# danihae/bio-image-unet

Hardware: AMD Instinct MI355X
Metric: voxels/sec fwd+bwd (higher is better)
Workload: dtype bf16; 1 GPU; cfg4: UNet3D(in_channels=1, out_channels=1, n_filter=32) input (4, 1, 128, 128, 128) per GPU, train step = forward + reference loss + backward + Adam; parallelism=dp1

## Files before the change

### bio_image_unet_amd/csrc/biu_api.hip

```cpp
#include "biu_common.h"
#include "biu_internal.h"

#include <stdlib.h>
#include <string.h>

static const char* const kOffTokens[] = {
    "conv_fwd", "conv_dgrad", "conv_wgrad", "convt_fwd", "convt_dgrad", "convt_wgrad", "convt_all", "c1", "c1_mfma", "cat",
    "fused_stats", "wgrad_bn", "dgrad_bnred", "pool_pair", "pool_pipe", "pool_bnred", "head_bnred", "ksplit", "m16", "m16x2", "rr16",
    "wroll", "wroll16", "wroll2d", "upconv", "foldt", "foldall", "foldck8", "foldgemm", "croll", "froll", "prepack", "wsplitbn",
    "capturefork", "sidechain", "headrank1",
};
constexpr int kNumOffTokens = sizeof(kOffTokens) / sizeof(kOffTokens[0]);
static_assert(kNumOffTokens <= 64, "BiuEnv::off holds one bit per token");

static int off_index(const char* tok, size_t n) {
    for (int i = 0; i < kNumOffTokens; ++i)
        if (strlen(kOffTokens[i]) == n && strncmp(kOffTokens[i], tok, n) == 0) return i;
    return -1;
}
static void env_unknown(const char* var, const char* val, int n) {
    fprintf(stderr, "[biu] %s: unknown %s '%.*s' ignored\n", var, strcmp(var, "BIU_DISABLE") == 0 ? "token" : "value", n, val);
}
static bool parse_int(const char* s, int* v) {
    char* end = nullptr;
    const long r = strtol(s, &end, 10);
    if (end == s || *end) return false;
    *v = (int)r;
    return true;
}

const BiuEnv& biu_env() {
    static const BiuEnv env = [] {
        BiuEnv v{0, false, false, 0, 2, 0, 128};
        if (const char* p = getenv("BIU_DISABLE")) {
            while (true) {
                const size_t n = strcspn(p, ",");
                const int i = off_index(p, n);
                if (i >= 0) v.off |= 1ull << i;
                else if (n > 0) env_unknown("BIU_DISABLE", p, (int)n);
                if (!p[n]) break;
                p += n + 1;
            }
        }
// ... 539 lines not shown
```

### bio_image_unet_amd/csrc/biu_c1.hip

```cpp
#include "biu_internal.h"
#include <stdlib.h>
#include <string.h>

namespace {

typedef float floatx16 __attribute__((ext_vector_type(16)));
typedef __bf16 bf16x8 __attribute__((ext_vector_type(8)));
typedef __bf16 bf16x4 __attribute__((ext_vector_type(4)));
typedef unsigned u32x2 __attribute__((ext_vector_type(2)));

constexpr int ROWB = 80;

struct C1Args {
    const char* x; int xpitch;
    char* y; int ypitch;
    const char* yraw; int yrawpitch;
    const float* w;
    const float* bias;
    const float* xs; const float* xb; const float* xl;
    int N, D, H, W, co0, cout;
    int nbd, nbh, nbw, nbricks;
    float* partial;
    int ctot;
    const float* bn_scale; const float* bn_shift; const float* bn_slope; const float* bn_cA; const float* bn_cB; const float* bn_cC;
};

__device__ __forceinline__ unsigned pack2(float a, float b) {
    typedef __bf16 bf2 __attribute__((ext_vector_type(2)));
    const bf2 p = {(__bf16)a, (__bf16)b};
    return __builtin_bit_cast(unsigned, p);
}
__device__ __forceinline__ void unpack8(const uint4& v, float* f) {
    const unsigned u[4] = {v.x, v.y, v.z, v.w};
#pragma unroll
    for (int i = 0; i < 4; ++i) { f[2 * i] = __uint_as_float(u[i] << 16); f[2 * i + 1] = __uint_as_float(u[i] & 0xffff0000u); }
}
__device__ __forceinline__ float bf2f(unsigned short u) { return __uint_as_float((unsigned)u << 16); }

template <int KD, int HALF = 0> struct Geo {
    static constexpr int TD = (KD == 3) ? (HALF ? 1 : 2) : 1, TH = (KD == 3) ? 8 : (HALF ? 8 : 16), TW = 32;
    static constexpr int BV = TD * TH * TW;
    static constexpr int HD = TD + KD - 1, HH = TH + 2, HW = TW + 2;
    static constexpr int HV = HD * HH * HW;
    static constexpr int TAPS = KD * 9;
};

template <int KD, int NTHR, int HALF = 0>
struct XpRegs { unsigned short v[(Geo<KD, HALF>::HV + NTHR - 1) / NTHR]; unsigned inside; };

template <int KD, int NTHR, int HALF = 0>
__device__ __forceinline__ void xp_request(const C1Args& a, int n, int d0, int h0, int w0, XpRegs<KD, NTHR, HALF>& xr) {
    using G = Geo<KD, HALF>;
    constexpr int NX = (G::HV + NTHR - 1) / NTHR;
    const int tid = threadIdx.x;
    xr.inside = 0;
#pragma unroll
    for (int k = 0; k < NX; ++k) {
        const int i = tid + NTHR * k;
        const int hw = i % G::HW, t = i / G::HW;
        const int hh = t % G::HH, hd = t / G::HH;
        const int gd = d0 + hd - (KD == 3 ? 1 : 0), gh = h0 + hh - 1, gw = w0 + hw - 1;
        const bool ok = i < G::HV && gd >= 0 && gd < a.D && gh >= 0 && gh < a.H && gw >= 0 && gw < a.W;
        xr.v[k] = ok ? *(const unsigned short*)(a.x + ((size_t)(((size_t)n * a.D + gd) * a.H + gh) * a.W + gw) * a.xpitch * 2) : (unsigned short)0;
        xr.inside |= ok ? (1u << k) : 0u;
    }
}
template <int KD, int NTHR, int HALF = 0>
__device__ __forceinline__ void xp_commit(const C1Args& a, const XpRegs<KD, NTHR, HALF>& xr, unsigned short* lx, char* lxp) {
    using G = Geo<KD, HALF>;
    constexpr int NX = (G::HV + NTHR - 1) / NTHR;
    const int tid = threadIdx.x;
    const bool has_xf = a.xs != nullptr;
    const float xs = has_xf ? a.xs[0] : 1.f, xb = has_xf ? a.xb[0] : 0.f, xl = has_xf ? a.xl[0] : 1.f;
#pragma unroll
    for (int k = 0; k < NX; ++k) {
        const int i = tid + NTHR * k;
        if (i < G::HV) {
            unsigned short v = xr.v[k];
            if (has_xf && ((xr.inside >> k) & 1u)) {
                const float tt = fmaf(xs, bf2f(v), xb);
                const float o = tt > 0.f ? tt : xl * tt;
                v = (unsigned short)(pack2(o, 0.f) & 0xffffu);
            }
            lx[i] = v;
        }
    }
    __syncthreads();
    for (int v = tid; v < G::BV; v += NTHR) {
        const int lw = v % G::TW, t = v / G::TW;
        const int lh = t % G::TH, ld = t / G::TH;
        unsigned short val[32];
#pragma unroll
        for (int tap = 0; tap < 32; ++tap) {
            if (tap < G::TAPS) {
                const int ta = tap / 9, tb = (tap / 3) % 3, tc = tap % 3;
                val[tap] = lx[((ld + ta) * G::HH + (lh + tb)) * G::HW + (lw + tc)];
            } else {
                val[tap] = 0;
            }
        }
        uint4* dst = (uint4*)(lxp + v * ROWB);
#pragma unroll
        for (int q = 0; q < 4; ++q)
            dst[q] = make_uint4(val[8 * q] | ((unsigned)val[8 * q + 1] << 16), val[8 * q + 2] | ((unsigned)val[8 * q + 3] << 16),
                                val[8 * q + 4] | ((unsigned)val[8 * q + 5] << 16), val[8 * q + 6] | ((unsigned)val[8 * q + 7] << 16));
    }
    __syncthreads();
}

template <int KD, int NQ >
__global__ __launch_bounds__(256) void k_c1_fwd_mfma(C1Args a) {
    using G = Geo<KD>;
    __shared__ __attribute__((aligned(16))) char smem[G::BV * ROWB + G::HV * 2 + 16 + 4 * 64 * 4 + 32 * 4];
    char* lxp = smem;
    unsigned short* lx = (unsigned short*)(smem + G::BV * ROWB);
    float* lred = (float*)(smem + G::BV * ROWB + ((G::HV * 2 + 15) & ~15));
    float* lbias = lred + 4 * 64;
    const int tid = threadIdx.x, lane = tid & 63, wave = tid >> 6, r = lane & 31, hf = lane >> 5;
    lred[tid] = 0.f;
    if (tid < 32) lbias[tid] = (a.bias && tid < a.cout) ? a.bias[a.co0 + tid] : 0.f;
    uint4 wf[2];
#pragma unroll
    for (int ks = 0; ks < 2; ++ks) {
        float f[8];
#pragma unroll
        for (int e = 0; e < 8; ++e) {
            const int tap = 16 * ks + 8 * hf + e;
            f[e] = (r < a.cout && tap < G::TAPS) ? a.w[(size_t)(a.co0 + r) * G::TAPS + tap] : 0.f;
        }
        wf[ks] = make_uint4(pack2(f[0], f[1]), pack2(f[2], f[3]), pack2(f[4], f[5]), pack2(f[6], f[7]));
    }
    float s1[NQ][8], s2[NQ][8];
#pragma unroll
    for (int q = 0; q < NQ; ++q)
#pragma unroll
        for (int e = 0; e < 8; ++e) s1[q][e] = s2[q][e] = 0.f;
    __syncthreads();

    auto origin_of = [&](int brick, int& n, int& d0, int& h0, int& w0) {
        int b = brick;
        w0 = (b % a.nbw) * G::TW; b /= a.nbw;
        h0 = (b % a.nbh) * G::TH; b /= a.nbh;
        d0 = (b % a.nbd) * G::TD;
        n = b / a.nbd;
    };
    XpRegs<KD, 256> xr;
    if ((int)blockIdx.x < a.nbricks) { int n, d0, h0, w0; origin_of(blockIdx.x, n, d0, h0, w0); xp_request<KD, 256>(a, n, d0, h0, w0, xr); }
    for (int brick = blockIdx.x; brick < a.nbricks; brick += gridDim.x) {
        int n, d0, h0, w0;
        origin_of(brick, n, d0, h0, w0);
        xp_commit<KD, 256>(a, xr, lx, lxp);
        if (brick + (int)gridDim.x < a.nbricks) { int n2, d2, h2, w2; origin_of(brick + gridDim.x, n2, d2, h2, w2); xp_request<KD, 256>(a, n2, d2, h2, w2, xr); }
        for (int tile = wave; tile < G::BV / 32; tile += 4) {
            const int v = tile * 32 + r;
            floatx16 acc;
#pragma unroll
            for (int e = 0; e < 16; ++e) acc[e] = lbias[8 * (e >> 2) + 4 * hf + (e & 3)];
#pragma unroll
            for (int ks = 0; ks < 2; ++ks) {
                const uint4 bx = *(const uint4*)(lxp + v * ROWB + (16 * ks + 8 * hf) * 2);
                acc = __builtin_amdgcn_mfma_f32_32x32x16_bf16(__builtin_bit_cast(bf16x8, wf[ks]), __builtin_bit_cast(bf16x8, bx), acc, 0, 0, 0);
            }
            const int lw = v % G::TW, t = v / G::TW;
            const int gd = d0 + t / G::TH, gh = h0 + t % G::TH, gw = w0 + lw;
            const bool vok = gd < a.D && gh < a.H && gw < a.W;
            char* orow = a.y + ((size_t)(((size_t)n * a.D + gd) * a.H + gh) * a.W + gw) * a.ypitch * 2;
#pragma unroll
            for (int q = 0; q < NQ; ++q) {
                unsigned a0 = pack2(acc[8 * q + 0], acc[8 * q + 1]), a1 = pack2(acc[8 * q + 2], acc[8 * q + 3]);
                unsigned b0 = pack2(acc[8 * q + 4], acc[8 * q + 5]), b1 = pack2(acc[8 * q + 6], acc[8 * q + 7]);
                const u32x2 r0 = __builtin_amdgcn_permlane32_swap(a0, b0, false, false);
                const u32x2 r1 = __builtin_amdgcn_permlane32_swap(a1, b1, false, false);
                const uint4 piece = make_uint4(r0[0], r1[0], r0[1], r1[1]);
                const int c = 16 * q + 8 * hf;
                if (vok && c < a.cout) {
                    *(uint4*)(orow + (size_t)(a.co0 + c) * 2) = piece;
                    float f[8];
                    unpack8(piece, f);
#pragma unroll
                    for (int e = 0; e < 8; ++e) { s1[q][e] += f[e]; s2[q][e] = fmaf(f[e], f[e], s2[q][e]); }
                }
            }
        }
        __syncthreads();
    }
    if (a.partial) {
#pragma unroll
        for (int q = 0; q < NQ; ++q)
#pragma unroll
            for (int e = 0; e < 8; ++e) {
                float u = s1[q][e], w_ = s2[q][e];
#pragma unroll
                for (int o = 16; o > 0; o >>= 1) { u += __shfl_xor(u, o, 64); w_ += __shfl_xor(w_, o, 64); }
                if (r == 0) { lred[wave * 64 + 2 * (16 * q + 8 * hf + e)] = u; lred[wave * 64 + 2 * (16 * q + 8 * hf + e) + 1] = w_; }
            }
        __syncthreads();
        if (tid < a.cout) {
            float* dst = a.partial + ((size_t)blockIdx.x * a.ctot + a.co0 + tid) * 2;
            dst[0] = (lred[2 * tid] + lred[64 + 2 * tid]) + (lred[128 + 2 * tid] + lred[192 + 2 * tid]);
            dst[1] = (lred[2 * tid + 1] + lred[64 + 2 * tid + 1]) + (lred[128 + 2 * tid + 1] + lred[192 + 2 * tid + 1]);
        }
    }
}

template <int KD>
__global__ __launch_bounds__(256, 3) void k_c1_wgrad_mfma(C1Args a) {
    using G = Geo<KD, 1>;
    constexpr int NTHR = 256, NWV = 4;
    extern __shared__ __attribute__((aligned(16))) char smem[];
    char* lxp = smem;
    char* ldy = smem + G::BV * ROWB;
    unsigned short* lx = (unsigned short*)(ldy + G::BV * ROWB);
    float* lacc = (float*)((char*)lx + ((G::HV * 2 + 15) & ~15));
    const int tid = threadIdx.x, lane = tid & 63, wave = tid >> 6;
    const bool fused = a.yraw != nullptr;
    const int ppv = a.cout / 8;
    const int mypiece = tid % 4;
    float ks[8], kh[8], kl[8], ka[8], kb[8], kc[8];
    if (fused && mypiece < ppv) {
#pragma unroll
        for (int e = 0; e < 8; ++e) {
            const int c = a.co0 + mypiece * 8 + e;
            ks[e] = a.bn_scale[c]; kh[e] = a.bn_shift[c]; kl[e] = a.bn_slope ? a.bn_slope[c] : 1.f;
            ka[e] = a.bn_cA[c]; kb[e] = a.bn_cB[c]; kc[e] = a.bn_cC[c];
        }
    }
    for (int i = tid; i < 32 * 32; i += NTHR) lacc[i] = 0.f;
    floatx16 acc;
#pragma unroll
    for (int e = 0; e < 16; ++e) acc[e] = 0.f;
    const int g = lane >> 4, li = lane & 15, qrow = li >> 2, p = li & 3, cg = g & 1, h = g >> 1;
    const int tr_lane = (8 * h + qrow) * ROWB + (16 * cg + 4 * p) * 2;

    constexpr int NPC = G::BV * 4 / NTHR;
    uint4 pda[NPC], pyr[NPC];
    size_t pvox[NPC];
    unsigned pmask = 0;
    auto origin = [&](int brick, int& n, int& d0, int& h0, int& w0) {
        int b = brick;
        w0 = (b % a.nbw) * G::TW; b /= a.nbw;
        h0 = (b % a.nbh) * G::TH; b /= a.nbh;
        d0 = (b % a.nbd) * G::TD;
        n = b / a.nbd;
    };
    auto request = [&](int brick) {
        int n, d0, h0, w0;
        origin(brick, n, d0, h0, w0);
        pmask = 0;
#pragma unroll
        for (int k = 0; k < NPC; ++k) {
            const int v = (tid + NTHR * k) / 4;
            const int lw = v % G::TW, t = v / G::TW;
            const int gd = d0 + t / G::TH, gh = h0 + t % G::TH, gw = w0 + lw;
            pda[k] = make_uint4(0, 0, 0, 0);
            pyr[k] = make_uint4(0, 0, 0, 0);
            if (mypiece < ppv && gd < a.D && gh < a.H && gw < a.W) {
                const size_t vox = (((size_t)n * a.D + gd) * a.H + gh) * a.W + gw;
                pvox[k] = vox;
                pda[k] = *(const uint4*)(a.y + (vox * a.ypitch + a.co0 + mypiece * 8) * 2);
                if (fused) pyr[k] = *(const uint4*)(a.yraw + (vox * a.yrawpitch + a.co0 + mypiece * 8) * 2);
                pmask |= 1u << k;
            }
        }
    };
    XpRegs<KD, NTHR, 1> xr;
    if ((int)blockIdx.x < a.nbricks) {
        request(blockIdx.x);
        int n0, d00, h00, w00;
        origin(blockIdx.x, n0, d00, h00, w00);
        xp_request<KD, NTHR, 1>(a, n0, d00, h00, w00, xr);
    }
    for (int brick = blockIdx.x; brick < a.nbricks; brick += gridDim.x) {
        int n, d0, h0, w0;
        origin(brick, n, d0, h0, w0);
#pragma unroll
        for (int k = 0; k < NPC; ++k) {
            const int v = (tid + NTHR * k) / 4;
            uint4 out = pda[k];
            if (fused && ((pmask >> k) & 1u)) {
                float gg[8], yy[8];
                unpack8(out, gg);
                unpack8(pyr[k], yy);
#pragma unroll
                for (int e = 0; e < 8; ++e) {
                    const float dz = gg[e] * (fmaf(ks[e], yy[e], kh[e]) > 0.f ? 1.f : kl[e]);
                    gg[e] = fmaf(ka[e], dz, fmaf(kb[e], yy[e], kc[e]));
                }
                out = make_uint4(pack2(gg[0], gg[1]), pack2(gg[2], gg[3]), pack2(gg[4], gg[5]), pack2(gg[6], gg[7]));
                *(uint4*)(a.y + (pvox[k] * a.ypitch + a.co0 + mypiece * 8) * 2) = out;
            }
            *(uint4*)(ldy + v * ROWB + mypiece * 16) = out;
        }
        xp_commit<KD, NTHR, 1>(a, xr, lx, lxp);
        if (brick + (int)gridDim.x < a.nbricks) {
            request(brick + gridDim.x);
            int n2, d2, h2, w2;
            origin(brick + gridDim.x, n2, d2, h2, w2);
            xp_request<KD, NTHR, 1>(a, n2, d2, h2, w2, xr);
        }
        typedef bf16x4 __attribute__((address_space(3))) * lp;
        for (int ksx = wave; ksx < G::BV / 16; ksx += NWV) {
            const char* ap = lxp + ksx * 16 * ROWB + tr_lane;
            const char* bp = ldy + ksx * 16 * ROWB + tr_lane;
            const bf16x4 a0 = __builtin_amdgcn_ds_read_tr16_b64_v4bf16((lp)(ap));
            const bf16x4 a1 = __builtin_amdgcn_ds_read_tr16_b64_v4bf16((lp)(ap + 4 * ROWB));
            const bf16x4 b0 = __builtin_amdgcn_ds_read_tr16_b64_v4bf16((lp)(bp));
            const bf16x4 b1 = __builtin_amdgcn_ds_read_tr16_b64_v4bf16((lp)(bp + 4 * ROWB));
            acc = __builtin_amdgcn_mfma_f32_32x32x16_bf16(__builtin_shufflevector(a0, a1, 0, 1, 2, 3, 4, 5, 6, 7),
                                                          __builtin_shufflevector(b0, b1, 0, 1, 2, 3, 4, 5, 6, 7), acc, 0, 0, 0);
        }
        __syncthreads();
    }
    {
        const int j = lane & 31, hf = lane >> 5;
#pragma unroll
        for (int e = 0; e < 16; ++e) atomicAdd(&lacc[((e & 3) + 8 * (e >> 2) + 4 * hf) * 32 + j], acc[e]);
    }
    __syncthreads();
    for (int i = tid; i < G::TAPS * a.cout; i += NTHR) {
        const int tap = i / a.cout, co = i % a.cout;
        a.partial[(size_t)blockIdx.x * (G::TAPS * a.cout) + i] = lacc[tap * 32 + co];
    }
}

__global__ void k_c1m_finalize(const float* __restrict__ partial, int nblk, int taps, int cout, int co0, float* __restrict__ dw) {
    __shared__ double red[256];
    const int o = blockIdx.x;
    double s = 0;
    for (int b = threadIdx.x; b < nblk; b += 256) s += partial[(size_t)b * (taps * cout) + o];
    red[threadIdx.x] = s;
    __syncthreads();
    for (int st = 128; st > 0; st >>= 1) {
        if (threadIdx.x < st) red[threadIdx.x] += red[threadIdx.x + st];
        __syncthreads();
    }
    if (threadIdx.x == 0) dw[(size_t)(co0 + o % cout) * taps + o / cout] = (float)red[0];
}

int cus() {
    static int n = 0;
    if (!n) {
        hipDeviceProp_t p;
        int dev = 0;
        if (hipGetDevice(&dev) == hipSuccess && hipGetDeviceProperties(&p, dev) == hipSuccess) n = p.multiProcessorCount;
        if (n <= 0) n = 256;
    }
    return n;
}

template <int KD, int HALF = 0> void bricks_of(C1Args& a) {
    using G = Geo<KD, HALF>;
    a.nbd = (a.D + G::TD - 1) / G::TD; a.nbh = (a.H + G::TH - 1) / G::TH; a.nbw = (a.W + G::TW - 1) / G::TW;
    a.nbricks = a.N * a.nbd * a.nbh * a.nbw;
}

}

bool biu_c1m_ok(const biu_act* x, const biu_act* y, int kd, int kh, int kw, int dil, int dtype) {
    if (biu_off("c1_mfma") || dtype != BIU_BF16 || x->c != 1 || dil != 1 || kh != 3 || kw != 3 || (kd != 1 && kd != 3)) return false;
    if (y->c % 16 != 0 || y->c < 16) return false;
    if ((uintptr_t)y->p % 16 || (y->pitch * 2) % 16 || (uintptr_t)x->p % 2) return false;
    return nvox(y) < (1LL << 31);
}

int biu_c1m_fwd_rows(const biu_act* y, int kd) {
    C1Args a{};
    a.N = y->n; a.D = y->d; a.H = y->h; a.W = y->w;
    if (kd == 3) bricks_of<3>(a); else bricks_of<1>(a);
    const int g = 3 * cus();
    return g < a.nbricks ? g : a.nbricks;
}

int biu_c1m_fwd(const biu_act* x, const biu_xform* xf, const float* w, const float* bias, int kd, const biu_act* y, float* bn_partial, hipStream_t st) {
    C1Args a{};
    a.x = (const char*)x->p; a.xpitch = x->pitch; a.y = (char*)y->p; a.ypitch = y->pitch; a.w = w; a.bias = bias;
    if (xf && (xf->scale || xf->shift || xf->slope)) {
        BIU_REQUIRE(xf->scale && xf->shift && xf->slope, BIU_ERR_UNSUPPORTED, "c1 conv: partial biu_xform");
        a.xs = xf->scale; a.xb = xf->shift; a.xl = xf->slope;
    }
    a.N = y->n; a.D = y->d; a.H = y->h; a.W = y->w; a.ctot = y->c; a.partial = bn_partial;
    const int rows = biu_c1m_fwd_rows(y, kd);
    if (kd == 3) bricks_of<3>(a); else bricks_of<1>(a);
    for (int co0 = 0; co0 < y->c;) {
        const int chunk = (y->c - co0) >= 32 ? 32 : 16;
        a.co0 = co0; a.cout = chunk;
        if (kd == 3) { if (chunk == 32) hipLaunchKernelGGL((k_c1_fwd_mfma<3, 2>), dim3(rows), dim3(256), 0, st, a); else hipLaunchKernelGGL((k_c1_fwd_mfma<3, 1>), dim3(rows), dim3(256), 0, st, a); }
        else { if (chunk == 32) hipLaunchKernelGGL((k_c1_fwd_mfma<1, 2>), dim3(rows), dim3(256), 0, st, a); else hipLaunchKernelGGL((k_c1_fwd_mfma<1, 1>), dim3(rows), dim3(256), 0, st, a); }
        co0 += chunk;
    }
    BIU_CHECK_LAUNCH("c1_fwd_mfma");
    return BIU_OK;
}

size_t biu_c1m_wgrad_workspace(int cout, int kd) { return (size_t)3 * cus() * kd * 9 * 32 * sizeof(float); }

int biu_c1m_wgrad(const biu_act* x, const biu_xform* xf, const biu_act* da, const BnBwdFuse* bn, int kd, float* dw, void* ws, size_t ws_bytes,
                  hipStream_t st) {
    BIU_REQUIRE(ws && ws_bytes >= biu_c1m_wgrad_workspace(da->c, kd), BIU_ERR_WORKSPACE, "c1_wgrad_mfma: workspace too small");
    C1Args a{};
    if (xf && (xf->scale || xf->shift || xf->slope)) {
        BIU_REQUIRE(xf->scale && xf->shift && xf->slope, BIU_ERR_UNSUPPORTED, "c1 conv: partial biu_xform");
        a.xs = xf->scale; a.xb = xf->shift; a.xl = xf->slope;
    }
    a.x = (const char*)x->p; a.xpitch = x->pitch; a.y = (char*)da->p; a.ypitch = da->pitch;
    a.N = da->n; a.D = da->d; a.H = da->h; a.W = da->w; a.partial = (float*)ws; a.ctot = da->c;
    if (bn) {
        a.yraw = (const char*)bn->y->p; a.yrawpitch = bn->y->pitch;
        a.bn_scale = bn->scale; a.bn_shift = bn->shift; a.bn_slope = bn->slope; a.bn_cA = bn->cA; a.bn_cB = bn->cB; a.bn_cC = bn->cC;
    }
    const int taps = kd * 9;
    if (kd == 3) bricks_of<3, 1>(a); else bricks_of<1, 1>(a);
    int grid = 3 * cus();
    if (grid > a.nbricks) grid = a.nbricks;
    const size_t hv = kd == 3 ? (size_t)Geo<3, 1>::HV : (size_t)Geo<1, 1>::HV;
    const size_t lds = (size_t)2 * 256 * ROWB + ((hv * 2 + 15) & ~(size_t)15) + 32 * 32 * sizeof(float);
    for (int co0 = 0; co0 < da->c;) {
        const int chunk = (da->c - co0) >= 32 ? 32 : 16;
        a.co0 = co0; a.cout = chunk;
        if (kd == 3) hipLaunchKernelGGL(k_c1_wgrad_mfma<3>, dim3(grid), dim3(256), lds, st, a);
        else hipLaunchKernelGGL(k_c1_wgrad_mfma<1>, dim3(grid), dim3(256), lds, st, a);
        BIU_CHECK_LAUNCH("c1_wgrad_mfma");
        hipLaunchKernelGGL(k_c1m_finalize, dim3(taps * chunk), dim3(256), 0, st, (const float*)ws, grid, taps, chunk, co0, dw);
        BIU_CHECK_LAUNCH("c1_wgrad_mfma_finalize");
        co0 += chunk;
    }
    return BIU_OK;
}
```

### bio_image_unet_amd/csrc/biu_special.hip

```cpp
#include "biu_internal.h"
#include <cstring>
#include <cstdlib>
#include <stdlib.h>

#define TPB 256

struct Vox4 { int n, d, h, w; };
__device__ __forceinline__ Vox4 unvox4(i64 v, int D, int H, int W) {
    Vox4 r;
    if ((unsigned long long)v < (1ull << 32)) {
        unsigned u = (unsigned)v;
        r.w = (int)(u % (unsigned)W); u /= (unsigned)W;
        r.h = (int)(u % (unsigned)H); u /= (unsigned)H;
        r.d = (int)(u % (unsigned)D); u /= (unsigned)D;
        r.n = (int)u;
        return r;
    }
    r.w = (int)(v % W); v /= W;
    r.h = (int)(v % H); v /= H;
    r.d = (int)(v % D); v /= D;
    r.n = (int)v;
    return r;
}

// ... 449 lines not shown
    BIU_CHECK_LAUNCH("bn_bwd_reduce_vec");
    return BIU_OK;
}

__global__ void k_partial_sum0(const float* __restrict__ partial, int nblk, int C, float* __restrict__ out) {
    __shared__ double red[TPB];
    const int c = blockIdx.x;
    double a = 0;
    for (int b = threadIdx.x; b < nblk; b += TPB) a += partial[((i64)b * C + c) * 2];
    red[threadIdx.x] = a;
    __syncthreads();
    for (int s = TPB / 2; s > 0; s >>= 1) {
        if (threadIdx.x < s) red[threadIdx.x] += red[threadIdx.x + s];
        __syncthreads();
    }
    if (threadIdx.x == 0) out[c] = (float)red[0];
}
size_t biu_chan_sum_workspace(int c) { return (size_t)BIU_BN_MAX_PARTIALS * c * 2 * sizeof(float); }
int biu_chan_sum_vec(const biu_act* a, float* out, void* ws, int dtype, hipStream_t st) {
    int nblk = 0;
    BIU_DISPATCH_DTYPE(dtype, {
        constexpr int PE = 16 / sizeof(T);
        VPlan p = vplan(nvox(a), a->c, PE);
        VSum<T> f{dact(a)};
        hipLaunchKernelGGL((k_chan_reduce2_vec<VSum<T>, PE>), dim3(p.nblk), dim3(TPB), p.smem, st, f, nvox(a), a->c, p.ppv, p.vpb, (float*)ws);
        nblk = p.nblk;
    });
    BIU_CHECK_LAUNCH("chan_sum_vec");
    hipLaunchKernelGGL(k_partial_sum0, dim3(a->c), dim3(TPB), 0, st, (const float*)ws, nblk, a->c, out);
    BIU_CHECK_LAUNCH("partial_sum0");
    return BIU_OK;
}

template <typename T, int C, int O, bool RED, bool STORE = true>
__global__ __launch_bounds__(TPB) void k_head_bwd_fused(DAct x, DXf xf, const float* __restrict__ w, int cout,
                                                        const float* __restrict__ dl, DAct dx, int want_dx,
                                                        float* __restrict__ partial ,
                                                        const float* __restrict__ mean, const float* __restrict__ invstd,
                                                        float* __restrict__ bn_partial) {
    constexpr int G = 16 / sizeof(T);
    __shared__ float wsm[O * C];
    __shared__ float xsc[C], xsh[C], xsl[C];
    __shared__ float red[4][O * C + O];
    for (int i = threadIdx.x; i < O * C; i += TPB) wsm[i] = (i / C) < cout ? w[i] : 0.f;
    for (int i = threadIdx.x; i < C; i += TPB) {
        xsc[i] = xf.scale ? xf.scale[i] : 1.f;
        xsh[i] = xf.shift ? xf.shift[i] : 0.f;
        xsl[i] = xf.slope ? xf.slope[i] : 1.f;
    }
    __syncthreads();
    const i64 S = (i64)x.d * x.h * x.w;
    const i64 total = (i64)x.n * S;
    float aw[O][C], ab[O];
    float r1[RED ? C : 1], r2[RED ? C : 1];
#pragma unroll
    for (int o = 0; o < O; ++o) {
        ab[o] = 0.f;
#pragma unroll
        for (int c = 0; c < C; ++c) aw[o][c] = 0.f;
    }
    if (RED) {
#pragma unroll
        for (int c = 0; c < C; ++c) r1[c] = r2[c] = 0.f;
    }
    for (i64 v = (i64)blockIdx.x * TPB + threadIdx.x; v < total; v += (i64)gridDim.x * TPB) {
        const i64 n = v / S, s = v % S;
        float g[O];
#pragma unroll
        for (int o = 0; o < O; ++o) {
            g[o] = (o < cout) ? dl[(n * cout + o) * S + s] : 0.f;
            ab[o] += g[o];
        }
        const T* src = (const T*)x.p + v * x.pitch;
        T* dst = (STORE && want_dx) ? (T*)dx.p + v * dx.pitch : nullptr;
#pragma unroll
        for (int c0 = 0; c0 < C; c0 += G) {
            Pack<T, G> in = *(const Pack<T, G>*)(src + c0);
            Pack<T, G> od;
#pragma unroll
            for (int j = 0; j < G; ++j) {
                const int c = c0 + j;
                float t = fmaf(xsc[c], to_f(in.v[j]), xsh[c]);
                t = t > 0.f ? t : xsl[c] * t;
                float d = 0.f;
#pragma unroll
                for (int o = 0; o < O; ++o) {
                    aw[o][c] = fmaf(g[o], t, aw[o][c]);
                    d = fmaf(g[o], wsm[o * C + c], d);
                }
                od.v[j] = from_f<T>(d);
                if (RED) {
                    const float yv = to_f(in.v[j]);
                    const float dz = to_f(od.v[j]) * (fmaf(xsc[c], yv, xsh[c]) > 0.f ? 1.f : xsl[c]);
                    r1[c] += dz;
                    r2[c] = fmaf(dz, yv, r2[c]);
                }
            }
            if (STORE && want_dx) *(Pack<T, G>*)(dst + c0) = od;
        }
    }
    const int lane = threadIdx.x & 63, wave = threadIdx.x >> 6;
#pragma unroll
    for (int o = 0; o < O; ++o) {
#pragma unroll
        for (int c = 0; c < C; ++c) {
            const float r = wave_sum(aw[o][c]);
            if (lane == 0) red[wave][o * C + c] = r;
        }
        const float rb = wave_sum(ab[o]);
        if (lane == 0) red[wave][O * C + o] = rb;
    }
    __syncthreads();
    for (int i = threadIdx.x; i < O * C + O; i += TPB)
        partial[(i64)blockIdx.x * (O * C + O) + i] = red[0][i] + red[1][i] + red[2][i] + red[3][i];
    if (RED) {
        __shared__ float redb[4][2 * C];
#pragma unroll
        for (int c = 0; c < C; ++c) {
            const float a1 = wave_sum(r1[c]), a2 = wave_sum(r2[c]);
            if (lane == 0) { redb[wave][2 * c] = a1; redb[wave][2 * c + 1] = a2; }
        }
        __syncthreads();
        for (int c = threadIdx.x; c < C; c += TPB) {
            const float s1v = redb[0][2 * c] + redb[1][2 * c] + redb[2][2 * c] + redb[3][2 * c];
            const float s2v = redb[0][2 * c + 1] + redb[1][2 * c + 1] + redb[2][2 * c + 1] + redb[3][2 * c + 1];
            bn_partial[((i64)blockIdx.x * C + c) * 2 + 0] = s1v;
            bn_partial[((i64)blockIdx.x * C + c) * 2 + 1] = invstd[c] * (s2v - mean[c] * s1v);
        }
    }
}

// ... 13 lines not shown
            const int o = i / C, c = i % C;
            if (o < cout && dw) dw[o * C + c] = (float)red[0];
        } else {
            const int o = i - O * C;
            if (o < cout && db) db[o] = (float)red[0];
        }
    }
}

#define HEAD_FUSED_BLOCKS 1024
bool biu_head_bwd_fused_ok(const biu_act* x, const biu_act* dx, int cout, int dtype) {
    const int c = x->c;
    if (!(c == 8 || c == 16 || c == 32 || c == 64)) return false;
    if (cout < 1 || cout > 4 || c * (cout == 3 ? 4 : cout) > 128) return false;
    const int g = 16 / (int)dsize(dtype);
    if (!vec_ok(x, g, dtype)) return false;
    if (dx && !vec_ok(dx, g, dtype)) return false;
    return true;
}
size_t biu_head_bwd_fused_workspace(int cin) { return (size_t)HEAD_FUSED_BLOCKS * (4 * cin + 4) * sizeof(float); }

template <typename T, int C>
static int head_fused_t(const biu_act* x, const biu_xform* xf, const float* w, int cout, const float* dl, const biu_act* dx, float* dw,
                        float* db, void* ws, hipStream_t st, const float* mean = nullptr, const float* invstd = nullptr,
                        float* bn_partial = nullptr, int* bn_nblk = nullptr) {
    const i64 total = nvox(x);
    int nblk = (int)((total + TPB * 8 - 1) / (TPB * 8));
    if (nblk > HEAD_FUSED_BLOCKS) nblk = HEAD_FUSED_BLOCKS;
    if (nblk < 1) nblk = 1;
    DAct dxa = dx ? dact(dx) : dact(x);
    const int O = cout == 3 ? 4 : cout;
    if (bn_partial) {
        if constexpr (C <= 32) {
            if (!dx) {
                if (O == 2) hipLaunchKernelGGL((k_head_bwd_fused<T, C, 2, true, false>), dim3(nblk), dim3(TPB), 0, st, dact(x), dxf(xf), w, cout, dl, dxa, 0, (float*)ws, mean, invstd, bn_partial);
                else hipLaunchKernelGGL((k_head_bwd_fused<T, C, 1, true, false>), dim3(nblk), dim3(TPB), 0, st, dact(x), dxf(xf), w, cout, dl, dxa, 0, (float*)ws, mean, invstd, bn_partial);
            } else if (O == 2) hipLaunchKernelGGL((k_head_bwd_fused<T, C, 2, true>), dim3(nblk), dim3(TPB), 0, st, dact(x), dxf(xf), w, cout, dl, dxa, 1, (float*)ws, mean, invstd, bn_partial);
            else hipLaunchKernelGGL((k_head_bwd_fused<T, C, 1, true>), dim3(nblk), dim3(TPB), 0, st, dact(x), dxf(xf), w, cout, dl, dxa, 1, (float*)ws, mean, invstd, bn_partial);
            *bn_nblk = nblk;
        }
    } else {
        if constexpr (C <= 32) {
            if (O == 4) hipLaunchKernelGGL((k_head_bwd_fused<T, C, 4, false>), dim3(nblk), dim3(TPB), 0, st, dact(x), dxf(xf), w, cout, dl, dxa, dx ? 1 : 0, (float*)ws, nullptr, nullptr, nullptr);
        }
        if (O == 2) hipLaunchKernelGGL((k_head_bwd_fused<T, C, 2, false>), dim3(nblk), dim3(TPB), 0, st, dact(x), dxf(xf), w, cout, dl, dxa, dx ? 1 : 0, (float*)ws, nullptr, nullptr, nullptr);
        if (O == 1) hipLaunchKernelGGL((k_head_bwd_fused<T, C, 1, false>), dim3(nblk), dim3(TPB), 0, st, dact(x), dxf(xf), w, cout, dl, dxa, dx ? 1 : 0, (float*)ws, nullptr, nullptr, nullptr);
    }
    BIU_CHECK_LAUNCH("head_bwd_fused");
    hipLaunchKernelGGL(k_head_bwd_finalize, dim3(O * C + O), dim3(TPB), 0, st, (const float*)ws, nblk, C, O, cout, dw, db);
    BIU_CHECK_LAUNCH("head_bwd_finalize");
    return BIU_OK;
}
bool biu_head_bwd_bnred_ok(const biu_act* x, const biu_act* dx, int cout, int dtype) {
    return x->c <= 32 && cout <= 2 && biu_head_bwd_fused_ok(x, dx, cout, dtype);
}
int biu_head_bwd_bnred_fused(const biu_act* x, const biu_xform* xf, const float* w, int cout, const float* dl, const biu_act* dx, float* dw,
                             float* db, void* ws, const float* mean, const float* invstd, float* bn_partial, int* bn_nblk, int dtype,
                             hipStream_t st) {
    BIU_DISPATCH_DTYPE(dtype, {
        switch (x->c) {
            case 8: return head_fused_t<T, 8>(x, xf, w, cout, dl, dx, dw, db, ws, st, mean, invstd, bn_partial, bn_nblk);
            case 16: return head_fused_t<T, 16>(x, xf, w, cout, dl, dx, dw, db, ws, st, mean, invstd, bn_partial, bn_nblk);
            default: return head_fused_t<T, 32>(x, xf, w, cout, dl, dx, dw, db, ws, st, mean, invstd, bn_partial, bn_nblk);
        }
    });
    return BIU_OK;
// ... 558 lines not shown
```

Measured before the change: 740.4 million voxels/s.

## Widen first-layer conv halo loads, pair im2col, pipeline head backward loads

Adds a 'c1wide' path to the first-layer (single-input-channel) conv forward and wgrad kernels. The halo is loaded as 32-bit pairs of voxels, and the im2col tile is built two voxels per thread from dword LDS reads, which cuts the number of scalar global and LDS accesses. The wgrad kernel swaps its LDS atomicAdd reduction for per-wave copies placed in the reused im2col buffer, and the forward kernel hoists the bias broadcast out of the tile loop. Separately, a 'headpipe' variant of the head backward kernel (bf16, 16 channels, one output) keeps weights and transform parameters in registers and double-buffers the next voxel's loads while the current one is reduced; this adds register pressure and code complexity.

```diff
diff --git a/bio_image_unet_amd/csrc/biu_api.hip b/bio_image_unet_amd/csrc/biu_api.hip
--- a/bio_image_unet_amd/csrc/biu_api.hip
+++ b/bio_image_unet_amd/csrc/biu_api.hip
@@ -8,7 +8,7 @@
     "conv_fwd", "conv_dgrad", "conv_wgrad", "convt_fwd", "convt_dgrad", "convt_wgrad", "convt_all", "c1", "c1_mfma", "cat",
     "fused_stats", "wgrad_bn", "dgrad_bnred", "pool_pair", "pool_pipe", "pool_bnred", "head_bnred", "ksplit", "m16", "m16x2", "rr16",
     "wroll", "wroll16", "wroll2d", "upconv", "foldt", "foldall", "foldck8", "foldgemm", "croll", "froll", "prepack", "wsplitbn",
-    "capturefork", "sidechain", "headrank1",
+    "capturefork", "sidechain", "headrank1", "c1wide", "headpipe",
 };
 constexpr int kNumOffTokens = sizeof(kOffTokens) / sizeof(kOffTokens[0]);
 static_assert(kNumOffTokens <= 64, "BiuEnv::off holds one bit per token");
diff --git a/bio_image_unet_amd/csrc/biu_c1.hip b/bio_image_unet_amd/csrc/biu_c1.hip
--- a/bio_image_unet_amd/csrc/biu_c1.hip
+++ b/bio_image_unet_amd/csrc/biu_c1.hip
@@ -46,14 +46,61 @@
 };
 
 template <int KD, int NTHR, int HALF = 0>
-struct XpRegs { unsigned short v[(Geo<KD, HALF>::HV + NTHR - 1) / NTHR]; unsigned inside; };
-
-template <int KD, int NTHR, int HALF = 0>
+struct XpRegs { unsigned v[(Geo<KD, HALF>::HV + NTHR - 1) / NTHR]; unsigned inside; };
+
+template <int KD, int HALF> struct GeoD {
+    using G = Geo<KD, HALF>;
+    static constexpr int ROWS = G::HD * G::HH, DPR = (G::TW + 4) / 2, ND = ROWS * DPR;
+};
+
+template <int KD, int HALF, int Q0, int Q1>
+__device__ __forceinline__ void im2col_pair(const unsigned* lx32, char* lxp, int pv) {
+    using G = Geo<KD, HALF>;
+    const int lw = 2 * (pv % (G::TW / 2)), t = pv / (G::TW / 2);
+    const int lh = t % G::TH, ld = t / G::TH;
+    constexpr int R0 = 8 * Q0 / 3, RL = (8 * Q1 - 1) / 3 < KD * 3 - 1 ? (8 * Q1 - 1) / 3 : KD * 3 - 1;
+    unsigned short va[33], vb[33];
+#pragma unroll
+    for (int i = 0; i < 33; ++i) va[i] = vb[i] = 0;
+#pragma unroll
+    for (int r = R0; r <= RL; ++r) {
+        const int idx = ((ld + r / 3) * G::HH + (lh + r % 3)) * G::HW + lw;
+        const unsigned e01 = lx32[idx >> 1], e23 = lx32[(idx >> 1) + 1];
+        va[3 * r] = (unsigned short)e01; va[3 * r + 1] = (unsigned short)(e01 >> 16); va[3 * r + 2] = (unsigned short)e23;
+        vb[3 * r] = (unsigned short)(e01 >> 16); vb[3 * r + 1] = (unsigned short)e23; vb[3 * r + 2] = (unsigned short)(e23 >> 16);
+    }
+    uint4* pa = (uint4*)(lxp + (2 * pv) * ROWB);
+    uint4* pb = (uint4*)(lxp + (2 * pv + 1) * ROWB);
+#pragma unroll
+    for (int q = Q0; q < Q1; ++q) {
+        pa[q] = make_uint4(va[8 * q] | ((unsigned)va[8 * q + 1] << 16), va[8 * q + 2] | ((unsigned)va[8 * q + 3] << 16),
+                           va[8 * q + 4] | ((unsigned)va[8 * q + 5] << 16), va[8 * q + 6] | ((unsigned)va[8 * q + 7] << 16));
+        pb[q] = make_uint4(vb[8 * q] | ((unsigned)vb[8 * q + 1] << 16), vb[8 * q + 2] | ((unsigned)vb[8 * q + 3] << 16),
+                           vb[8 * q + 4] | ((unsigned)vb[8 * q + 5] << 16), vb[8 * q + 6] | ((unsigned)vb[8 * q + 7] << 16));
+    }
+}
+
+template <int KD, int NTHR, int HALF, int WIDE>
 __device__ __forceinline__ void xp_request(const C1Args& a, int n, int d0, int h0, int w0, XpRegs<KD, NTHR, HALF>& xr) {
     using G = Geo<KD, HALF>;
-    constexpr int NX = (G::HV + NTHR - 1) / NTHR;
+    using GD = GeoD<KD, HALF>;
+    constexpr int NX = (G::HV + NTHR - 1) / NTHR, NXD = (GD::ND + NTHR - 1) / NTHR;
+    static_assert(NXD <= NX && G::HW % 2 == 0 && G::TW % 2 == 0, "the dword form shares the per-voxel form's registers");
     const int tid = threadIdx.x;
     xr.inside = 0;
+    if constexpr (WIDE & 2) {
+#pragma unroll
+        for (int k = 0; k < NXD; ++k) {
+            const int i = tid + NTHR * k;
+            const int j = i % GD::DPR, row = i / GD::DPR;
+            const int hh = row % G::HH, hd = row / G::HH;
+            const int gd = d0 + hd - (KD == 3 ? 1 : 0), gh = h0 + hh - 1, gw = w0 - 2 + 2 * j;
+            const bool ok = i < GD::ND && gd >= 0 && gd < a.D && gh >= 0 && gh < a.H && gw >= 0 && gw < a.W;
+            xr.v[k] = ok ? *(const unsigned*)(a.x + ((size_t)(((size_t)n * a.D + gd) * a.H + gh) * a.W + gw) * 2) : 0u;
+            xr.inside |= ok ? (1u << k) : 0u;
+        }
+        return;
+    }
 #pragma unroll
     for (int k = 0; k < NX; ++k) {
         const int i = tid + NTHR * k;
@@ -61,31 +108,58 @@
         const int hh = t % G::HH, hd = t / G::HH;
         const int gd = d0 + hd - (KD == 3 ? 1 : 0), gh = h0 + hh - 1, gw = w0 + hw - 1;
         const bool ok = i < G::HV && gd >= 0 && gd < a.D && gh >= 0 && gh < a.H && gw >= 0 && gw < a.W;
-        xr.v[k] = ok ? *(const unsigned short*)(a.x + ((size_t)(((size_t)n * a.D + gd) * a.H + gh) * a.W + gw) * a.xpitch * 2) : (unsigned short)0;
+        xr.v[k] = ok ? *(const unsigned short*)(a.x + ((size_t)(((size_t)n * a.D + gd) * a.H + gh) * a.W + gw) * a.xpitch * 2) : 0u;
         xr.inside |= ok ? (1u << k) : 0u;
     }
 }
-template <int KD, int NTHR, int HALF = 0>
+template <int KD, int NTHR, int HALF, int WIDE>
 __device__ __forceinline__ void xp_commit(const C1Args& a, const XpRegs<KD, NTHR, HALF>& xr, unsigned short* lx, char* lxp) {
     using G = Geo<KD, HALF>;
-    constexpr int NX = (G::HV + NTHR - 1) / NTHR;
+    using GD = GeoD<KD, HALF>;
+    constexpr int NX = (G::HV + NTHR - 1) / NTHR, NXD = (GD::ND + NTHR - 1) / NTHR;
     const int tid = threadIdx.x;
     const bool has_xf = a.xs != nullptr;
     const float xs = has_xf ? a.xs[0] : 1.f, xb = has_xf ? a.xb[0] : 0.f, xl = has_xf ? a.xl[0] : 1.f;
-#pragma unroll
-    for (int k = 0; k < NX; ++k) {
-        const int i = tid + NTHR * k;
-        if (i < G::HV) {
-            unsigned short v = xr.v[k];
-            if (has_xf && ((xr.inside >> k) & 1u)) {
-                const float tt = fmaf(xs, bf2f(v), xb);
-                const float o = tt > 0.f ? tt : xl * tt;
-                v = (unsigned short)(pack2(o, 0.f) & 0xffffu);
-            }
-            lx[i] = v;
+    auto xform = [&](unsigned short v) {
+        const float tt = fmaf(xs, bf2f(v), xb);
+        const float o = tt > 0.f ? tt : xl * tt;
+        return (unsigned short)(pack2(o, 0.f) & 0xffffu);
+    };
+    if constexpr (WIDE & 2) {
+#pragma unroll
+        for (int k = 0; k < NXD; ++k) {
+            const int i = tid + NTHR * k;
+            if (i < GD::ND) {
+                const int j = i % GD::DPR, row = i / GD::DPR;
+                unsigned short lo = (unsigned short)(xr.v[k] & 0xffffu), hi = (unsigned short)(xr.v[k] >> 16);
+                if (has_xf && ((xr.inside >> k) & 1u)) { lo = xform(lo); hi = xform(hi); }
+                if (j > 0) lx[row * G::HW + 2 * j - 1] = lo;
+                if (j < GD::DPR - 1) lx[row * G::HW + 2 * j] = hi;
+            }
+        }
+    } else {
+#pragma unroll
+        for (int k = 0; k < NX; ++k) {
+            const int i = tid + NTHR * k;
+            if (i < G::HV) {
+                unsigned short v = (unsigned short)xr.v[k];
+                if (has_xf && ((xr.inside >> k) & 1u)) v = xform(v);
+                lx[i] = v;
+            }
         }
     }
     __syncthreads();
+    if constexpr (WIDE & 1) {
+        const unsigned* lx32 = (const unsigned*)lx;
+        if constexpr (KD == 3 && G::BV / 2 * 2 == NTHR) {
+            const int pv = tid % (G::BV / 2);
+            if (tid < G::BV / 2) im2col_pair<KD, HALF, 0, 2>(lx32, lxp, pv); else im2col_pair<KD, HALF, 2, 4>(lx32, lxp, pv);
+        } else {
+            for (int pv = tid; pv < G::BV / 2; pv += NTHR) im2col_pair<KD, HALF, 0, 4>(lx32, lxp, pv);
+        }
+        __syncthreads();
+        return;
+    }
     for (int v = tid; v < G::BV; v += NTHR) {
         const int lw = v % G::TW, t = v / G::TW;
         const int lh = t % G::TH, ld = t / G::TH;
@@ -108,7 +182,7 @@
     __syncthreads();
 }
 
-template <int KD, int NQ >
+template <int KD, int NQ , int WIDE >
 __global__ __launch_bounds__(256) void k_c1_fwd_mfma(C1Args a) {
     using G = Geo<KD>;
     __shared__ __attribute__((aligned(16))) char smem[G::BV * ROWB + G::HV * 2 + 16 + 4 * 64 * 4 + 32 * 4];
@@ -144,18 +218,19 @@
         d0 = (b % a.nbd) * G::TD;
         n = b / a.nbd;
     };
+    floatx16 bias16;
+#pragma unroll
+    for (int e = 0; e < 16; ++e) bias16[e] = lbias[8 * (e >> 2) + 4 * hf + (e & 3)];
     XpRegs<KD, 256> xr;
-    if ((int)blockIdx.x < a.nbricks) { int n, d0, h0, w0; origin_of(blockIdx.x, n, d0, h0, w0); xp_request<KD, 256>(a, n, d0, h0, w0, xr); }
+    if ((int)blockIdx.x < a.nbricks) { int n, d0, h0, w0; origin_of(blockIdx.x, n, d0, h0, w0); xp_request<KD, 256, 0, WIDE>(a, n, d0, h0, w0, xr); }
     for (int brick = blockIdx.x; brick < a.nbricks; brick += gridDim.x) {
         int n, d0, h0, w0;
         origin_of(brick, n, d0, h0, w0);
-        xp_commit<KD, 256>(a, xr, lx, lxp);
-        if (brick + (int)gridDim.x < a.nbricks) { int n2, d2, h2, w2; origin_of(brick + gridDim.x, n2, d2, h2, w2); xp_request<KD, 256>(a, n2, d2, h2, w2, xr); }
+        xp_commit<KD, 256, 0, WIDE>(a, xr, lx, lxp);
+        if (brick + (int)gridDim.x < a.nbricks) { int n2, d2, h2, w2; origin_of(brick + gridDim.x, n2, d2, h2, w2); xp_request<KD, 256, 0, WIDE>(a, n2, d2, h2, w2, xr); }
         for (int tile = wave; tile < G::BV / 32; tile += 4) {
             const int v = tile * 32 + r;
-            floatx16 acc;
-#pragma unroll
-            for (int e = 0; e < 16; ++e) acc[e] = lbias[8 * (e >> 2) + 4 * hf + (e & 3)];
+            floatx16 acc = bias16;
 #pragma unroll
             for (int ks = 0; ks < 2; ++ks) {
                 const uint4 bx = *(const uint4*)(lxp + v * ROWB + (16 * ks + 8 * hf) * 2);
@@ -203,7 +278,7 @@
     }
 }
 
-template <int KD>
+template <int KD, int WIDE>
 __global__ __launch_bounds__(256, 3) void k_c1_wgrad_mfma(C1Args a) {
     using G = Geo<KD, 1>;
     constexpr int NTHR = 256, NWV = 4;
@@ -211,7 +286,6 @@
     char* lxp = smem;
     char* ldy = smem + G::BV * ROWB;
     unsigned short* lx = (unsigned short*)(ldy + G::BV * ROWB);
-    float* lacc = (float*)((char*)lx + ((G::HV * 2 + 15) & ~15));
     const int tid = threadIdx.x, lane = tid & 63, wave = tid >> 6;
     const bool fused = a.yraw != nullptr;
     const int ppv = a.cout / 8;
@@ -225,7 +299,6 @@
             ka[e] = a.bn_cA[c]; kb[e] = a.bn_cB[c]; kc[e] = a.bn_cC[c];
         }
     }
-    for (int i = tid; i < 32 * 32; i += NTHR) lacc[i] = 0.f;
     floatx16 acc;
 #pragma unroll
     for (int e = 0; e < 16; ++e) acc[e] = 0.f;
@@ -268,7 +341,7 @@
         request(blockIdx.x);
         int n0, d00, h00, w00;
         origin(blockIdx.x, n0, d00, h00, w00);
-        xp_request<KD, NTHR, 1>(a, n0, d00, h00, w00, xr);
+        xp_request<KD, NTHR, 1, WIDE>(a, n0, d00, h00, w00, xr);
     }
     for (int brick = blockIdx.x; brick < a.nbricks; brick += gridDim.x) {
         int n, d0, h0, w0;
@@ -291,12 +364,12 @@
             }
             *(uint4*)(ldy + v * ROWB + mypiece * 16) = out;
         }
-        xp_commit<KD, NTHR, 1>(a, xr, lx, lxp);
+        xp_commit<KD, NTHR, 1, WIDE>(a, xr, lx, lxp);
         if (brick + (int)gridDim.x < a.nbricks) {
             request(brick + gridDim.x);
             int n2, d2, h2, w2;
             origin(brick + gridDim.x, n2, d2, h2, w2);
-            xp_request<KD, NTHR, 1>(a, n2, d2, h2, w2, xr);
+            xp_request<KD, NTHR, 1, WIDE>(a, n2, d2, h2, w2, xr);
         }
         typedef bf16x4 __attribute__((address_space(3))) * lp;
         for (int ksx = wave; ksx < G::BV / 16; ksx += NWV) {
@@ -311,15 +384,17 @@
         }
         __syncthreads();
     }
+    static_assert(NWV * 32 * 32 * sizeof(float) <= (size_t)G::BV * ROWB, "the per-wave copies fit the im2col tile");
+    float* lacc = (float*)lxp;
     {
         const int j = lane & 31, hf = lane >> 5;
 #pragma unroll
-        for (int e = 0; e < 16; ++e) atomicAdd(&lacc[((e & 3) + 8 * (e >> 2) + 4 * hf) * 32 + j], acc[e]);
+        for (int e = 0; e < 16; ++e) lacc[wave * 1024 + ((e & 3) + 8 * (e >> 2) + 4 * hf) * 32 + j] = acc[e];
     }
     __syncthreads();
     for (int i = tid; i < G::TAPS * a.cout; i += NTHR) {
-        const int tap = i / a.cout, co = i % a.cout;
-        a.partial[(size_t)blockIdx.x * (G::TAPS * a.cout) + i] = lacc[tap * 32 + co];
+        const int tap = i / a.cout, co = i % a.cout, o = tap * 32 + co;
+        a.partial[(size_t)blockIdx.x * (G::TAPS * a.cout) + i] = (lacc[o] + lacc[1024 + o]) + (lacc[2048 + o] + lacc[3072 + o]);
     }
 }
 
@@ -348,6 +423,22 @@
     return n;
 }
 
+int wide_of(const biu_act* x, int W) {
+    if (biu_off("c1wide")) return 0;
+    return 1 | ((x->pitch == 1 && (uintptr_t)x->p % 4 == 0 && W % 2 == 0) ? 2 : 0);
+}
+
+template <int KD, int NQ> void launch_fwd(const C1Args& a, int wide, int rows, hipStream_t st) {
+    if (wide == 3) hipLaunchKernelGGL((k_c1_fwd_mfma<KD, NQ, 3>), dim3(rows), dim3(256), 0, st, a);
+    else if (wide == 1) hipLaunchKernelGGL((k_c1_fwd_mfma<KD, NQ, 1>), dim3(rows), dim3(256), 0, st, a);
+    else hipLaunchKernelGGL((k_c1_fwd_mfma<KD, NQ, 0>), dim3(rows), dim3(256), 0, st, a);
+}
+template <int KD> void launch_wgrad(const C1Args& a, int wide, int grid, size_t lds, hipStream_t st) {
+    if (wide == 3) hipLaunchKernelGGL((k_c1_wgrad_mfma<KD, 3>), dim3(grid), dim3(256), lds, st, a);
+    else if (wide == 1) hipLaunchKernelGGL((k_c1_wgrad_mfma<KD, 1>), dim3(grid), dim3(256), lds, st, a);
+    else hipLaunchKernelGGL((k_c1_wgrad_mfma<KD, 0>), dim3(grid), dim3(256), lds, st, a);
+}
+
 template <int KD, int HALF = 0> void bricks_of(C1Args& a) {
     using G = Geo<KD, HALF>;
     a.nbd = (a.D + G::TD - 1) / G::TD; a.nbh = (a.H + G::TH - 1) / G::TH; a.nbw = (a.W + G::TW - 1) / G::TW;
@@ -379,13 +470,14 @@
         a.xs = xf->scale; a.xb = xf->shift; a.xl = xf->slope;
     }
     a.N = y->n; a.D = y->d; a.H = y->h; a.W = y->w; a.ctot = y->c; a.partial = bn_partial;
+    const int wide = wide_of(x, y->w);
     const int rows = biu_c1m_fwd_rows(y, kd);
     if (kd == 3) bricks_of<3>(a); else bricks_of<1>(a);
     for (int co0 = 0; co0 < y->c;) {
         const int chunk = (y->c - co0) >= 32 ? 32 : 16;
         a.co0 = co0; a.cout = chunk;
-        if (kd == 3) { if (chunk == 32) hipLaunchKernelGGL((k_c1_fwd_mfma<3, 2>), dim3(rows), dim3(256), 0, st, a); else hipLaunchKernelGGL((k_c1_fwd_mfma<3, 1>), dim3(rows), dim3(256), 0, st, a); }
-        else { if (chunk == 32) hipLaunchKernelGGL((k_c1_fwd_mfma<1, 2>), dim3(rows), dim3(256), 0, st, a); else hipLaunchKernelGGL((k_c1_fwd_mfma<1, 1>), dim3(rows), dim3(256), 0, st, a); }
+        if (kd == 3) { if (chunk == 32) launch_fwd<3, 2>(a, wide, rows, st); else launch_fwd<3, 1>(a, wide, rows, st); }
+        else { if (chunk == 32) launch_fwd<1, 2>(a, wide, rows, st); else launch_fwd<1, 1>(a, wide, rows, st); }
         co0 += chunk;
     }
     BIU_CHECK_LAUNCH("c1_fwd_mfma");
@@ -404,6 +496,7 @@
     }
     a.x = (const char*)x->p; a.xpitch = x->pitch; a.y = (char*)da->p; a.ypitch = da->pitch;
     a.N = da->n; a.D = da->d; a.H = da->h; a.W = da->w; a.partial = (float*)ws; a.ctot = da->c;
+    const int wide = wide_of(x, da->w);
     if (bn) {
         a.yraw = (const char*)bn->y->p; a.yrawpitch = bn->y->pitch;
         a.bn_scale = bn->scale; a.bn_shift = bn->shift; a.bn_slope = bn->slope; a.bn_cA = bn->cA; a.bn_cB = bn->cB; a.bn_cC = bn->cC;
@@ -413,12 +506,11 @@
     int grid = 3 * cus();
     if (grid > a.nbricks) grid = a.nbricks;
     const size_t hv = kd == 3 ? (size_t)Geo<3, 1>::HV : (size_t)Geo<1, 1>::HV;
-    const size_t lds = (size_t)2 * 256 * ROWB + ((hv * 2 + 15) & ~(size_t)15) + 32 * 32 * sizeof(float);
+    const size_t lds = (size_t)2 * 256 * ROWB + ((hv * 2 + 15) & ~(size_t)15);
     for (int co0 = 0; co0 < da->c;) {
         const int chunk = (da->c - co0) >= 32 ? 32 : 16;
         a.co0 = co0; a.cout = chunk;
-        if (kd == 3) hipLaunchKernelGGL(k_c1_wgrad_mfma<3>, dim3(grid), dim3(256), lds, st, a);
-        else hipLaunchKernelGGL(k_c1_wgrad_mfma<1>, dim3(grid), dim3(256), lds, st, a);
+        if (kd == 3) launch_wgrad<3>(a, wide, grid, lds, st); else launch_wgrad<1>(a, wide, grid, lds, st);
         BIU_CHECK_LAUNCH("c1_wgrad_mfma");
         hipLaunchKernelGGL(k_c1m_finalize, dim3(taps * chunk), dim3(256), 0, st, (const float*)ws, grid, taps, chunk, co0, dw);
         BIU_CHECK_LAUNCH("c1_wgrad_mfma_finalize");
diff --git a/bio_image_unet_amd/csrc/biu_special.hip b/bio_image_unet_amd/csrc/biu_special.hip
--- a/bio_image_unet_amd/csrc/biu_special.hip
+++ b/bio_image_unet_amd/csrc/biu_special.hip
@@ -505,7 +505,7 @@
     return BIU_OK;
 }
 
-template <typename T, int C, int O, bool RED, bool STORE = true>
+template <typename T, int C, int O, bool RED, bool STORE = true, bool PIPE = false>
 __global__ __launch_bounds__(TPB) void k_head_bwd_fused(DAct x, DXf xf, const float* __restrict__ w, int cout,
                                                         const float* __restrict__ dl, DAct dx, int want_dx,
                                                         float* __restrict__ partial ,
@@ -536,40 +536,98 @@
 #pragma unroll
         for (int c = 0; c < C; ++c) r1[c] = r2[c] = 0.f;
     }
-    for (i64 v = (i64)blockIdx.x * TPB + threadIdx.x; v < total; v += (i64)gridDim.x * TPB) {
-        const i64 n = v / S, s = v % S;
-        float g[O];
-#pragma unroll
-        for (int o = 0; o < O; ++o) {
-            g[o] = (o < cout) ? dl[(n * cout + o) * S + s] : 0.f;
-            ab[o] += g[o];
-        }
-        const T* src = (const T*)x.p + v * x.pitch;
-        T* dst = (STORE && want_dx) ? (T*)dx.p + v * dx.pitch : nullptr;
-#pragma unroll
-        for (int c0 = 0; c0 < C; c0 += G) {
-            Pack<T, G> in = *(const Pack<T, G>*)(src + c0);
-            Pack<T, G> od;
-#pragma unroll
-            for (int j = 0; j < G; ++j) {
-                const int c = c0 + j;
-                float t = fmaf(xsc[c], to_f(in.v[j]), xsh[c]);
-                t = t > 0.f ? t : xsl[c] * t;
-                float d = 0.f;
-#pragma unroll
-                for (int o = 0; o < O; ++o) {
-                    aw[o][c] = fmaf(g[o], t, aw[o][c]);
-                    d = fmaf(g[o], wsm[o * C + c], d);
+    if constexpr (PIPE) {
+        static_assert(O == 1, "one head channel: dl[(n * cout + o) * S + s] is dl[v]");
+        float ksc[C], ksh[C], ksl[C], kw[C];
+#pragma unroll
+        for (int c = 0; c < C; ++c) {
+            ksc[c] = xf.scale ? xf.scale[c] : 1.f;
+            ksh[c] = xf.shift ? xf.shift[c] : 0.f;
+            ksl[c] = xf.slope ? xf.slope[c] : 1.f;
+            kw[c] = cout > 0 ? w[c] : 0.f;
+        }
+        struct Ld { Pack<T, G> in[C / G]; float g; };
+        auto issue = [&](i64 v, Ld& l) {
+            l.g = dl[v];
+            const T* src = (const T*)x.p + v * x.pitch;
+#pragma unroll
+            for (int c0 = 0; c0 < C; c0 += G) l.in[c0 / G] = *(const Pack<T, G>*)(src + c0);
+        };
+        auto reduce = [&](i64 v, const Ld& l) {
+            ab[0] += l.g;
+            T* dst = (STORE && want_dx) ? (T*)dx.p + v * dx.pitch : nullptr;
+#pragma unroll
+            for (int c0 = 0; c0 < C; c0 += G) {
+                const Pack<T, G>& in = l.in[c0 / G];
+                Pack<T, G> od;
+#pragma unroll
+                for (int j = 0; j < G; ++j) {
+                    const int c = c0 + j;
+                    float t = fmaf(ksc[c], to_f(in.v[j]), ksh[c]);
+                    t = t > 0.f ? t : ksl[c] * t;
+                    float d = 0.f;
+                    aw[0][c] = fmaf(l.g, t, aw[0][c]);
+                    d = fmaf(l.g, kw[c], d);
+                    od.v[j] = from_f<T>(d);
+                    if (RED) {
+                        const float yv = to_f(in.v[j]);
+                        const float dz = to_f(od.v[j]) * (fmaf(ksc[c], yv, ksh[c]) > 0.f ? 1.f : ksl[c]);
+                        r1[c] += dz;
+                        r2[c] = fmaf(dz, yv, r2[c]);
+                    }
                 }
-                od.v[j] = from_f<T>(d);
-                if (RED) {
-                    const float yv = to_f(in.v[j]);
-                    const float dz = to_f(od.v[j]) * (fmaf(xsc[c], yv, xsh[c]) > 0.f ? 1.f : xsl[c]);
-                    r1[c] += dz;
-                    r2[c] = fmaf(dz, yv, r2[c]);
+                if (STORE && want_dx) *(Pack<T, G>*)(dst + c0) = od;
+            }
+        };
+        const i64 vstep = (i64)gridDim.x * TPB;
+        i64 v = (i64)blockIdx.x * TPB + threadIdx.x;
+        if (v < total) {
+            Ld l0, l1;
+            issue(v, l0);
+            auto stage = [&](const Ld& cur, Ld& fill) {
+                if (v + vstep < total) issue(v + vstep, fill);
+                reduce(v, cur);
+                v += vstep;
+                return v < total;
+            };
+            while (stage(l0, l1) && stage(l1, l0)) {}
+        }
+    } else {
+        for (i64 v = (i64)blockIdx.x * TPB + threadIdx.x; v < total; v += (i64)gridDim.x * TPB) {
+            const i64 n = v / S, s = v % S;
+            float g[O];
+    #pragma unroll
+            for (int o = 0; o < O; ++o) {
+                g[o] = (o < cout) ? dl[(n * cout + o) * S + s] : 0.f;
+                ab[o] += g[o];
+            }
+            const T* src = (const T*)x.p + v * x.pitch;
+            T* dst = (STORE && want_dx) ? (T*)dx.p + v * dx.pitch : nullptr;
+    #pragma unroll
+            for (int c0 = 0; c0 < C; c0 += G) {
+                Pack<T, G> in = *(const Pack<T, G>*)(src + c0);
+                Pack<T, G> od;
+    #pragma unroll
+                for (int j = 0; j < G; ++j) {
+                    const int c = c0 + j;
+                    float t = fmaf(xsc[c], to_f(in.v[j]), xsh[c]);
+                    t = t > 0.f ? t : xsl[c] * t;
+                    float d = 0.f;
+    #pragma unroll
+                    for (int o = 0; o < O; ++o) {
+                        aw[o][c] = fmaf(g[o], t, aw[o][c]);
+                        d = fmaf(g[o], wsm[o * C + c], d);
+                    }
+                    od.v[j] = from_f<T>(d);
+                    if (RED) {
+                        const float yv = to_f(in.v[j]);
+                        const float dz = to_f(od.v[j]) * (fmaf(xsc[c], yv, xsh[c]) > 0.f ? 1.f : xsl[c]);
+                        r1[c] += dz;
+                        r2[c] = fmaf(dz, yv, r2[c]);
+                    }
                 }
-            }
-            if (STORE && want_dx) *(Pack<T, G>*)(dst + c0) = od;
+                if (STORE && want_dx) *(Pack<T, G>*)(dst + c0) = od;
+            }
         }
     }
     const int lane = threadIdx.x & 63, wave = threadIdx.x >> 6;
@@ -649,6 +707,17 @@
     const int O = cout == 3 ? 4 : cout;
     if (bn_partial) {
         if constexpr (C <= 32) {
+            if constexpr (sizeof(T) == 2 && C == 16) {
+                if (O == 1 && !biu_off("headpipe")) {
+                    if (!dx) hipLaunchKernelGGL((k_head_bwd_fused<T, C, 1, true, false, true>), dim3(nblk), dim3(TPB), 0, st, dact(x), dxf(xf), w, cout, dl, dxa, 0, (float*)ws, mean, invstd, bn_partial);
+                    else hipLaunchKernelGGL((k_head_bwd_fused<T, C, 1, true, true, true>), dim3(nblk), dim3(TPB), 0, st, dact(x), dxf(xf), w, cout, dl, dxa, 1, (float*)ws, mean, invstd, bn_partial);
+                    *bn_nblk = nblk;
+                    BIU_CHECK_LAUNCH("head_bwd_fused");
+                    hipLaunchKernelGGL(k_head_bwd_finalize, dim3(O * C + O), dim3(TPB), 0, st, (const float*)ws, nblk, C, O, cout, dw, db);
+                    BIU_CHECK_LAUNCH("head_bwd_finalize");
+                    return BIU_OK;
+                }
+            }
             if (!dx) {
                 if (O == 2) hipLaunchKernelGGL((k_head_bwd_fused<T, C, 2, true, false>), dim3(nblk), dim3(TPB), 0, st, dact(x), dxf(xf), w, cout, dl, dxa, 0, (float*)ws, mean, invstd, bn_partial);
                 else hipLaunchKernelGGL((k_head_bwd_fused<T, C, 1, true, false>), dim3(nblk), dim3(TPB), 0, st, dact(x), dxf(xf), w, cout, dl, dxa, 0, (float*)ws, mean, invstd, bn_partial);
```

Measured after the change: 744.0 million voxels/s, median of 6. No clear change (+0.5%).
